# FlowEternal/multitask-hydranet

Hardware: AMD Instinct MI355X
Metric: images/sec (fwd+bwd) HydraNet @ default res, 1/2/4/8 MI355X; CPU-ref same run (higher is better)
Workload: dtype bf16; 1 GPU; full HydraNet (backbone + BiFPN + seg/det/lane heads + multitask loss), big cfg, fwd+loss+bwd; batch_per_gpu=16, global_batch=16, resolution=3x512x1024, parallelism=dp1, hipgraph=True

## Files before the change

include/hydranet_hip.h:

```cpp
#ifndef HYDRANET_HIP_H
#define HYDRANET_HIP_H

#ifdef __cplusplus
extern "C" {
#endif

typedef struct ihipStream_t* hipStream_t;


int hn_gconv_pack_diag(const float* w, void* wk, void* wd, int C, hipStream_t stream);
int hn_pack_weight(const float* w, void* wp, void* wt, int Cout, int Cin, int taps, hipStream_t stream);
int hn_pack_weight_ex(const float* w, void* wp, void* wt, int Cout, int Cin_total, int ci0, int Cin, int taps, int phase, const float* bias,
                      float* b_eff, hipStream_t stream);
int hn_phase_fold(const float* dw_eff, const float* dw1, const float* db_eff, float* dw, float* db, int K, int C0, int C1, hipStream_t stream);
int hn_pack_weights_batched(const long* jobs, int njobs, long total_blocks, const int* block_job, hipStream_t stream);
int hn_pack_small_batched(const long* jobs, const int* block_job, long total_blocks, hipStream_t stream);

int hn_conv_gemm_nt(const void* x0, const void* x1, int mode, int n_img, int H, int W, int C0, int C1, int ld0, int ld1, int up, long M,
                    const void* w, int Nout, int KP, int taps, const float* bias, int act, void* out, int out_f32, int ldc, long rpi,
                    long img_stride, float* psum, float* psq, hipStream_t stream);
int hn_nt_stat_rows(long M, int Nout);
int hn_nt_stat_tile(long M, int Nout);
int hn_direct_stat_rows(int n_img, int H, int W);
int hn_conv_gemm_nt_imgw(const void* x0, int ld0, long M, int C0, const void* w, long w_img_stride, long rows_per_image, int Nout, int KP,
                         const float* bias, int act, void* out, int ldc, const void* addend, int ld_add, hipStream_t stream);
int hn_scale_weight_gate(const void* wp, const float* gate, void* out, int N, int Cout, int C, int KP, hipStream_t stream);
int hn_conv_gemm_nt_lvl(const void* x0, int ld0, long M, int C0, const void* w, int Nout, int KP, const float* bias, int act, void* out,
                        int ldc, const float* coef, int nlev, const long* rows, hipStream_t stream);
int hn_conv_gemm_nt_lvlout(const void* x0, int ld0, long M, int C0, const void* w, int Nout, int KP, const float* bias, int act, float* out,
                           int ldc, long img_stride, int n_img, int nlev, const int* H, const int* W, int row_align, hipStream_t stream);

int hn_conv_gemm_nt_ex(const void* x0, const void* x1, int mode, int n_img, int H, int W, int C0, int C1, int ld0, int ld1, int up, long M,
                       const void* w, int Nout, int KP, int taps, const float* bias, int act, void* out, int out_f32, int ldc, long rpi,
                       long img_stride, float* psum, float* psq, const float* xscale, const float* xshift, const float* xgate, long xhw,
                       int xact, const void* addend, int ld_add, int add_mode, hipStream_t stream);
int hn_conv_gemm_nt_stat(const void* x0, const void* x1, int mode, int n_img, int H, int W, int C0, int C1, int ld0, int ld1, int up, long M,
                         const void* w, int Nout, int KP, int taps, const float* bias, int act, void* out, int out_f32, int ldc, long rpi,
                         long img_stride, float* psum, float* psq, const void* addend, int ld_add, int add_mode, int emode, const void* ez,
                         int ld_ez, const float* ecoef, hipStream_t stream);
int hn_conv_gemm_nt_stat3(const void* x0, int ld0, long M, int C0, const void* w, int Nout, int KP, void* out, int ldc, float* psum, float* psq,
                          const void* addend, int ld_add, const void* ez, int ld_ez, const void* ey, int ld_ey, const float* ecoef,
                          hipStream_t stream);
int hn_wgrad_plan(int mode, int n_img, int H, int W, long M, int Nout, int KP, int taps, int* splits, long* rows_per_split, long* ws_bytes);
int hn_conv_gemm_tn(const void* x0, const void* x1, int mode, int n_img, int H, int W, int C0, int C1, int ld0, int ld1, int up, long M,
                    const void* dz, int ldz, int Nout, int KP, int taps, float* workspace, float* dw, hipStream_t stream);


int hn_stem_fwd(const float* x, const float* w, void* z, void* patches, int N, int H, int W, hipStream_t stream);

int hn_gconv_pack(const float* w, void* wk, void* wd, int C, int flip, hipStream_t stream);
int hn_gconv_fwd(const void* in, int ldi, const void* wk, void* out, int ldo, int N, int Hi, int Wi, int C, int stride, hipStream_t stream);
int hn_gconv_dgrad_s2(const void* dz, int ldz, const void* wd, void* dx, int ldx, int N, int Hi, int Wi, int C, hipStream_t stream);
long hn_wgrad_chunks(long pixels, long items);
int hn_gconv_wgrad(const void* x, int ldx, const void* dz, int ldz, float* part, int N, int Hi, int Wi, int C, int stride,
                   hipStream_t stream);

int hn_dw_pack(const float* w, void* wk, void* wkf, int C, hipStream_t stream);
int hn_dwconv_fwd(const void* in, int ldi, const void* wk, void* out, int ldo, int N, int H, int W, int C, hipStream_t stream);
int hn_dwconv_fwd_levels(const void* in, int ldi, const void* wk, void* out, int ldo, int N, int C, int nlev, const int* H, const int* W,
                         int row_align, int accumulate, hipStream_t stream);
long hn_dwconv_wgrad_blocks(long strips, int C);
int hn_dwconv_wgrad(const void* x, int ldx, const void* dz, int ldz, float* part, int N, int H, int W, int C, hipStream_t stream);
int hn_dwconv_wgrad_levels(const void* x, int ldx, const void* dz, int ldz, float* part, int N, int C, int nlev, const int* H, const int* W,
                           int row_align, hipStream_t stream);
long hn_dwconv_bwd_blocks(long strips, int C);
long hn_dwconv_bwd_blocks_levels(int N, int C, int nlev, const int* H, const int* W);
int hn_dwconv_bwd_levels(const void* dz, int ldz, const void* x, int ldx, const void* wf, void* dx, int lddx, float* part, int N, int C,
                         int nlev, const int* H, const int* W, int row_align, int accumulate, hipStream_t stream);

int hn_maxpool_fwd(const void* in, int ldi, void* out, int ldo, int N, int H, int W, int C, int mode, hipStream_t stream);
int hn_maxpool_bwd(const void* in, int ldi, const void* dout, int ldd, void* dx, int ldx, const float* wscale, int N, int H, int W, int C,
                   int mode, hipStream_t stream);
int hn_maxpool_bwd2(const void* in, int ldi, const void* dout, int ldd, void* dx, int ldx, const float* wscale, void* arg_ws, int N, int H,
                    int W, int C, int mode, int accumulate, hipStream_t stream);

int hn_up2_fwd(const void* in, int ldi, void* out, int ldo, int N, int H, int W, int C, hipStream_t stream);
int hn_sum2x2(const void* g, int ldg, void* out, int ldo, const float* wscale, int N, int H, int W, int C, int accumulate, hipStream_t stream);

int hn_fuse_dweights(const float* pw, int blocks, const float* praw, int nw, float eps, float* dp, hipStream_t stream);
int hn_fuse_fwd(const void* const* in, const int* ld, const int* mode, const float* w, void* out, int ldo, int N, int H, int W, int C,
                hipStream_t stream);
int hn_fuse_fwd_raw(const void* const* in, const int* ld, const int* mode, const float* praw, int nw, float eps, float* wn, void* out, int ldo,
                    int N, int H, int W, int C, hipStream_t stream);
int hn_fuse_bwd_blocks(int N, int H, int W, int C);
int hn_fuse_bwd(const void* const* in, const int* ld, const int* mode, const float* w, const void* dout, int ldd, void* g, int ldg,
                void* const* din, const int* ldin, const int* acc, float* pw, int N, int H, int W, int C, hipStream_t stream);
int hn_fuse_bwd_arg(const void* const* in, const int* ld, const int* mode, const float* w, const void* dout, int ldd, void* g, int ldg,
                    void* const* din, const int* ldin, const int* acc, float* pw, void* const* arg_out, int N, int H, int W, int C,
                    hipStream_t stream);
int hn_maxpool_bwd_from_arg(const void* arg, const void* dout, int ldd, void* dx, int ldx, const float* wscale, int N, int H, int W, int C,
                            int mode, int accumulate, hipStream_t stream);

long hn_fold_ring_rows(int H, int W);
int hn_conv3x3_dgrad_fold(const void* dz, int ldz, int Cz, int n_img, int H, int W, const void* wt, int Nout, int KP, int phase_k, int clamp,
                          void* out, int ldo, const void* yprev, int ldy, void* ring, hipStream_t stream);
int hn_conv3x3_dgrad_fold_s2d(const void* dz, int ldz, int Cz, int n_img, int H, int W, const void* wt, int Nout, int KP, int phase_k, int clamp,
                              void* out, int ldo, void* out_s2d, int ld_s2d, const void* yprev, int ldy, void* ring, hipStream_t stream);
int hn_seg_fold(const void* dvp, int ldv, int c0, void* out, int ldo, const void* yprev, int ldy, int N, int H, int W, int C, int up,
                hipStream_t stream);

int hn_space_to_depth(const float* dy, void* out, int ldo, int N, int h, int w, int k, hipStream_t stream);

int hn_space_to_depth_blocks(int N, int h, int w, int k);
int hn_space_to_depth_bf16(const void* in, int ldi, void* out, int N, int h, int w, int k, float* psum, hipStream_t stream);

// ... 260 lines not shown
```

multitask_hydranet_amd/csrc/hn_gemm.hip:

```cpp
#include "hn_common.h"
#include <climits>

#ifdef HN_TUNING
#define HN_DBG(p) ((p).dbg)
#else
#define HN_DBG(p) 0
#endif

struct XSrc {
    const bf16* x0;
    const bf16* x1;
    int mode;
    int H, W;
    int Hi, Wi;
    int C0, C1;
    int ld0, ld1;
    int up;
    long M;
    int clamp;
    int diag;
};

__device__ __forceinline__ int border_idx(int v, int L, int clamp) {
    if (clamp == 2) return (v < 0 || v >= L) ? -1 : v;
// ... 610 lines not shown
    if (staged || want_stats) __syncthreads();
    if (want_stats && !e3 && tid < BC && c_blk + tid < p.Nout) {
        const float* red = reinterpret_cast<const float*>(smem + BP * BC * 2);
        float t1 = 0.f, t2 = 0.f;
#pragma unroll
        for (int k = 0; k < WGP; ++k) { t1 += red[(k * BC + tid) * 2]; t2 += red[(k * BC + tid) * 2 + 1]; }
        p.psum[(long)p_tile * p.Nout + c_blk + tid] = t1;
        if (p.psq) p.psq[(long)p_tile * p.Nout + c_blk + tid] = t2;
    }
    if (staged) {
        bf16* outp = reinterpret_cast<bf16*>(p.out);
        float e1[8], e2[8], emu[8], ers[8];
#pragma unroll
        for (int k = 0; k < 8; ++k) { e1[k] = 0.f; e2[k] = 0.f; emu[k] = 0.f; ers[k] = 0.f; }
        if (e3) {
            const int co = c_blk + (tid % NPC) * 8;
            if (co < p.Nout) {
#pragma unroll
                for (int k = 0; k < 8; ++k) { emu[k] = p.ecoef[2 * p.Nout + co + k]; ers[k] = p.ecoef[3 * p.Nout + co + k]; }
            }
        }
#pragma unroll
        for (int u = 0; u < NIT; ++u) {
            const int idx = tid + 256 * u;
            if (idx >= BP * NPC) break;
            const int row = idx / NPC, pc = idx % NPC;
            const long pix = p_blk + row;
            const int co = c_blk + pc * 8;
            if (pix < p.x.M && co < p.Nout) {
                bf16x8 v = *reinterpret_cast<const bf16x8*>(smem + row * (BC * 2) + (((pc ^ row) & (NPC - 1)) << 4));
                long orow = pix * p.ldc;
                if (p.rpi) {
                    const unsigned im = (unsigned)pix / (unsigned)p.rpi;
                    orow = (long)im * p.img_stride + (long)((unsigned)pix - im * (unsigned)p.rpi) * p.ldc;
                }
                if (p.addend && !p.add_pre) {
                    bool has = true;
                    bf16x8 a;
                    if (PRE) {
                        has = phas[u < PRE ? u : 0];
                        a = padd[u < PRE ? u : 0];
                    } else {
                        long arow = pix;
                        if (p.add_s2) {
                            const unsigned W = (unsigned)p.x.W, H = (unsigned)p.x.H;
                            const unsigned x = (unsigned)pix % W, t = (unsigned)pix / W;
                            const unsigned y = t % H, n = t / H;
                            has = !((x | y) & 1u);
                            arow = ((long)n * (H >> 1) + (y >> 1)) * (W >> 1) + (x >> 1);
                        }
                        a = has ? ld8(p.addend + arow * p.ld_add + co) : zero8();
                    }
                    if (has) {
#pragma unroll
                        for (int k = 0; k < 8; ++k) v[k] = f2bf(bf2f(v[k]) + bf2f(a[k]));
                    }
                }
                if (e3) {
                    const bf16x8 yv = PRE ? pey[u < PRE ? u : 0] : ld8(p.ey + pix * p.ld_ey + co);
                    const bf16x8 zv = PRE ? pzz[u < PRE ? u : 0] : ld8(p.ez + pix * p.ld_ez + co);
#pragma unroll
                    for (int k = 0; k < 8; ++k) {
                        const float g = bf2f(yv[k]) > 0.f ? bf2f(v[k]) : 0.f;
                        e1[k] += g;
                        e2[k] += g * (bf2f(zv[k]) - emu[k]) * ers[k];
                    }
                }
                *reinterpret_cast<bf16x8*>(outp + orow + co) = v;
            }
        }
        if (e3) {
            float* r3 = reinterpret_cast<float*>(smem + BP * BC * 2 + WGP * BC * 8);
            static_assert(BP * BC * 2 + WGP * BC * 8 + 256 * 16 * 4 <= R * KG * STAGE || BC < 64, "emode 3 scratch fits the operand ring");
#pragma unroll
            for (int k = 0; k < 8; ++k) { r3[tid * 16 + k] = e1[k]; r3[tid * 16 + 8 + k] = e2[k]; }
            __syncthreads();
            if (tid < BC && c_blk + tid < p.Nout) {
                const int pc = tid >> 3, k = tid & 7;
                float t1 = 0.f, t2 = 0.f;
                for (int j = 0; j < 256 / NPC; ++j) { t1 += r3[(j * NPC + pc) * 16 + k]; t2 += r3[(j * NPC + pc) * 16 + 8 + k]; }
                p.psum[(long)p_tile * p.Nout + c_blk + tid] = t1;
                p.psq[(long)p_tile * p.Nout + c_blk + tid] = t2;
            }
        }
    }
}

template <int BC, bool OUT_F32, bool PIPE, int XB = (PIPE ? 2 : 1)>
__global__ __launch_bounds__(512, 4) void conv3x3_direct_kernel(const GemmNT p) {
    constexpr int KC = PIPE ? 32 : 64;
    constexpr int NPP = KC / 8, PB = KC * 2;
    constexpr int XBUFS = XB, WBUFS = PIPE ? 4 : 2;
    constexpr int WCO = BC >= 64 ? 64 : BC;
    constexpr int WGC = BC / WCO, WGP = 8 / WGC, ROWS = 16 / WGP;
    constexpr int TC = WCO / 16, TP = ROWS;
    constexpr int PPIX = 18 * 18, XL = (PPIX * NPP + 511) / 512, WL = (BC * NPP + 511) / 512;
    constexpr bool PRE32 = PIPE && XB == 1;
    constexpr int XBYTES = PIPE ? XL * 512 * 16 : (PPIX * 128 + 1023) / 1024 * 1024, WBYTES = PRE32 ? BC * PB : (PIPE ? WL * 512 * 16 : BC * 128);
    extern __shared__ __attribute__((aligned(16))) char smem[];
    char* sXb = smem;
    char* sWb = smem + XBUFS * XBYTES;
    const int tid = threadIdx.x, lane = tid & 63, wave = __builtin_amdgcn_readfirstlane(tid >> 6);
    const int wc = wave / WGP, wp = wave % WGP;
    const XSrc& xs = p.x;
    const int ncy = (p.Nout + BC - 1) / BC;
    const int tx_n = (xs.W + 15) >> 4, ty_n = (xs.H + 15) >> 4;
    const int lid = xcd_remap(blockIdx.x, gridDim.x);
    unsigned long long* stampb = (HN_DBG(p) & 16) && (blockIdx.x & 63) == 0 && tid == 0
                                     ? reinterpret_cast<unsigned long long*>(p.dbg_buf) + (blockIdx.x >> 6) * 128 : nullptr;
    int stampi = 0;
    auto stamp = [&]() {
#ifdef HN_TUNING
        __builtin_amdgcn_sched_barrier(0);
        if (stampb && stampi < 128) stampb[stampi++] = __builtin_amdgcn_s_memtime();
        __builtin_amdgcn_sched_barrier(0);
#endif
    };
    stamp();
    const int npatch = gridDim.x / ncy;
    const int c_tile = p.tile_major ? lid / npatch : lid % ncy;
    int t = p.tile_major ? lid % npatch : lid / ncy;
    const int patch_id = t;
    const int tx = t % tx_n;
    t /= tx_n;
    const int ty = t % ty_n;
    const int n = t / ty_n;
    const int c_blk = c_tile * BC, oy0 = ty * 16, ox0 = tx * 16;
    const int org = xs.mode == 2 ? -1 : -2;
    const int Ctot = xs.C0 + xs.C1;
    const int NT = p.phase_mode ? 4 : 9;
    const int nchunk = xs.diag ? 1 : (p.KP + KC - 1) / KC, S = nchunk * NT;
    const int Ktot = 9 * p.KP;
    const int tile_phase = p.phase_mode == 1 ? c_blk / p.phase_span : 0;
    const int cpp = p.phase_mode == 2 ? p.phase_span / KC : 0;
    struct Cur { int chunk, ti, ph, cnt; };
    auto cur0 = [&]() { Cur c; c.chunk = 0; c.ti = 0; c.ph = tile_phase; c.cnt = 0; return c; };
    auto adv = [&](Cur& c) {
        if (++c.ti == NT) {
            c.ti = 0;
            ++c.chunk;
            if (p.phase_mode == 2 && ++c.cnt == cpp) { c.cnt = 0; ++c.ph; }
        }
    };
    auto tap_at = [&](const Cur& c) { return p.phase_mode ? ((c.ph >> 1) + (c.ti >> 1)) * 3 + (c.ph & 1) + (c.ti & 1) : c.ti; };
    const int xc0 = xs.diag ? c_blk : 0;
    float* sbias = reinterpret_cast<float*>(smem + XBUFS * XBYTES + ((!PIPE || PRE32) && p.wpre ? S : WBUFS) * WBYTES);
    if (tid < BC) sbias[tid] = (p.bias && c_blk + tid < p.Nout) ? p.bias[c_blk + tid] : 0.f;

    if (BC == 64 && !PIPE && xs.diag) {
#pragma unroll
        for (int i = 0; i < 2; ++i) {
            if (512 * i + 64 * wave < 9 * 64) {
                const int e = 512 * i + tid, tap = e >> 6, col = e & 63, co = c_blk + col;
                const bf16* src = co < p.Nout ? p.w + co * (9 * p.KP) + tap * 64 + (col >> 3) * 8 : g_zero_piece;
                glds16(src, smem + XBUFS * XBYTES + (512 * i + 64 * wave) * 16);
            }
        }
    }
    int* patch_src = reinterpret_cast<int*>(sbias + BC);
    if (tid < 36) {
        const bool isy = tid < 18;
        const int k = isy ? tid : tid - 18, L = isy ? xs.Hi : xs.Wi;
        int g = (isy ? oy0 : ox0) + org + k;
        if (xs.mode == 2) g = border_idx(g, L, xs.clamp);
        else g = (g >= 0 && g < L) ? g : -1;
        patch_src[tid] = g;
// ... 2147 lines not shown
    const XSrc& x = p.x;
    const long npatch = (long)cdiv(x.W, 16) * cdiv(x.H, 16) * n_img;
    if (x.clamp == 1 && !x.diag && !out_f32 && p.d2s == 64 && p.phase_mode == 1 && p.phase_span == 64 && p.taps == 9 && p.KP == 64 && x.C0 == 64 &&
        x.C1 == 0 && p.Nout == 256 && !p.psum && !p.addend && (p.act == HN_ACT_ELU || p.act == HN_ACT_NONE) && (x.ld0 & 7) == 0 &&
        (p.ldc & 7) == 0 && p.ldc >= 64 && aligned16(p.out) && g_hn_knob[11] != 3 && npatch >= 1024) {
        SegPhase q;
        q.x = x.x0; q.ldx = x.ld0; q.N = n_img; q.H = x.H; q.W = x.W; q.w = p.w; q.bias = p.bias; q.out = (bf16*)p.out; q.ldc = p.ldc;
        q.act = p.act; q.npatch = (int)npatch;
        q.ppw = cdiv(npatch, 64);
        const int grid = 4 * cdiv(npatch, q.ppw);
        const size_t lds = 2 * (size_t)((18 * 18 * 8 + 63) / 64) * 1024 + 256 * 128;
        static std::atomic<unsigned long long> optin_sp{0};
        if (!lds_optin(optin_sp, {(const void*)seg_phase64_conv_kernel})) return HN_ERR_LAUNCH;
        hipLaunchKernelGGL(seg_phase64_conv_kernel, dim3(grid), dim3(512), lds, st, q);
        HN_LAUNCH_CHECK();
    }
    if (x.clamp == 1 && !x.diag && out_f32 && p.d2s && p.taps == 9 && p.KP == 64 && x.C0 == 64 && x.C1 == 0 && p.Nout == 4 * p.d2s &&
        p.Nout <= 32 && !p.psum && !p.addend && p.phase_mode == 0 && p.act == HN_ACT_NONE && (x.ld0 & 7) == 0 && ((32 * p.d2s) & 3) == 0 &&
        ((2 * x.W * p.d2s) & 3) == 0 && aligned16(p.out) && g_hn_knob[11] != 3 && npatch >= 1024) {
        SegOut q;
        q.x = x.x0; q.ldx = x.ld0; q.N = n_img; q.H = x.H; q.W = x.W; q.w = p.w; q.Nout = p.Nout; q.k = p.d2s; q.bias = p.bias;
        q.out = p.amax ? nullptr : (float*)p.out; q.amax = p.amax; q.npatch = (int)npatch;
        q.ppw = cdiv(npatch, 256);
        const int grid = cdiv(npatch, q.ppw);
        const size_t lds = 2 * (size_t)((18 * 18 * 8 + 63) / 64) * 1024 + (size_t)32 * 32 * p.d2s * 4;
        static std::atomic<unsigned long long> optin_so{0};
        if (!lds_optin(optin_so, {(const void*)seg_out_conv_kernel<true>, (const void*)seg_out_conv_kernel<false>})) return HN_ERR_LAUNCH;
        if (p.amax) hipLaunchKernelGGL(seg_out_conv_kernel<true>, dim3(grid), dim3(512), lds, st, q);
        else hipLaunchKernelGGL(seg_out_conv_kernel<false>, dim3(grid), dim3(512), lds, st, q);
        HN_LAUNCH_CHECK();
    }
    HN_CHECK_ARG(x.Wi < 8192 && x.Hi < 32768);
    int bc = x.diag ? 64 : (p.Nout <= 16 ? 16 : (p.Nout <= 32 ? 32 : (p.Nout <= 64 ? 64 : 128)));
    if (p.phase_mode == 1 && p.phase_span < bc) bc = 64;
    const bool staged_ok = (p.ldc & 7) == 0 && (p.Nout & 7) == 0 && aligned16(p.out) && (!p.d2s || ((p.d2s & 7) == 0 && p.Nout % bc == 0));
    if (bc >= 64 && !out_f32 && !staged_ok) {
        if (x.diag) return HN_ERR_UNSUPPORTED;
        bc = 32;
    }
    dim3 grid((unsigned)(cdiv(p.Nout, bc) * cdiv(x.W, 16) * cdiv(x.H, 16) * n_img));
    const int nsteps = p.phase_mode ? 4 : 9;
    p.wpre = (!x.diag && p.KP <= 64 && (size_t)nsteps * bc * 128 <= 32768 && g_hn_knob[11] != 2) ? 1 : 0;
    const bool narrow = bc == 64 && !out_f32 && !x.diag && !p.wpre && p.KP <= 32 && nsteps == 9 && g_hn_knob[18] == 0;
    if (narrow) p.wpre = 1;
#ifdef HN_TUNING
    const bool pipe = narrow || (g_direct_pipe && bc >= 64 && !out_f32 && !x.diag && !p.wpre && p.KP > 64);
#else
    const bool pipe = narrow;
#endif
    const size_t lds = narrow ? (size_t)(((18 * 18 * 4 + 511) / 512) * 512 * 16) + 9 * (size_t)(64 * 64)
                     : pipe ? (size_t)2 * (((18 * 18 * 4 + 511) / 512) * 512 * 16) + 4 * (size_t)(512 * 16)
                            : (size_t)((18 * 18 * 128 + 1023) / 1024 * 1024) + (p.wpre ? nsteps : 2) * (size_t)bc * 128;
    const size_t lds_bias = (size_t)bc * 4 + 36 * 4;
    static std::atomic<unsigned long long> optin{0};
    if (!lds_optin(optin, {(const void*)conv3x3_direct_kernel<16, true, false>, (const void*)conv3x3_direct_kernel<16, false, false>,
                           (const void*)conv3x3_direct_kernel<32, true, false>, (const void*)conv3x3_direct_kernel<32, false, false>,
                           (const void*)conv3x3_direct_kernel<64, true, false>, (const void*)conv3x3_direct_kernel<64, false, false>,
                           (const void*)conv3x3_direct_kernel<128, true, false>, (const void*)conv3x3_direct_kernel<128, false, false>}))
        return HN_ERR_LAUNCH;
    if (narrow) {
        hipLaunchKernelGGL((conv3x3_direct_kernel<64, false, true, 1>), grid, dim3(512), lds + lds_bias, st, p);
        HN_LAUNCH_CHECK();
    }
#ifdef HN_TUNING
    static std::atomic<unsigned long long> optin_pipe{0};
    if (pipe) {
        if (!lds_optin(optin_pipe, {(const void*)conv3x3_direct_kernel<64, false, true>, (const void*)conv3x3_direct_kernel<128, false, true>}))
            return HN_ERR_LAUNCH;
        if (bc == 64) hipLaunchKernelGGL((conv3x3_direct_kernel<64, false, true>), grid, dim3(512), lds + lds_bias, st, p);
        else hipLaunchKernelGGL((conv3x3_direct_kernel<128, false, true>), grid, dim3(512), lds + lds_bias, st, p);
        HN_LAUNCH_CHECK();
    }
#endif
#define DIRECT_CASE(BC_) \
    if (bc == BC_) { \
        if (out_f32) hipLaunchKernelGGL((conv3x3_direct_kernel<BC_, true, false>), grid, dim3(512), lds + lds_bias, st, p); \
        else hipLaunchKernelGGL((conv3x3_direct_kernel<BC_, false, false>), grid, dim3(512), lds + lds_bias, st, p); \
    }
    DIRECT_CASE(16) DIRECT_CASE(32) DIRECT_CASE(64) DIRECT_CASE(128)
#undef DIRECT_CASE
    HN_LAUNCH_CHECK();
}

static int run_gemm_nt(GemmNT& p, int n_img, bool out_f32, hipStream_t st) {
    const XSrc& x = p.x;
    const int Nout = p.Nout, KP = p.KP, taps = p.taps;
    const long M = x.M;
    HN_CHECK_ARG(x.x0 && p.w && p.out && M > 0 && Nout > 0 && KP > 0 && (KP & 31) == 0 && taps >= 1 && taps <= 9);
    HN_CHECK_ARG(!p.xscale || (p.xshift && x.mode <= 1 && !out_f32 && x.C1 == 0 && (!p.xgate || p.xhw > 0)));
    HN_CHECK_ARG(p.phase_mode == 0 || ((x.mode == 3 || x.clamp == 1) && p.phase_span >= 64 && p.phase_span % 64 == 0 && !p.psum && !p.rpi));
    HN_CHECK_ARG(!p.addend || p.add_pre || (!out_f32 && (Nout & 7) == 0 && (p.ldc & 7) == 0 && (p.ld_add & 7) == 0 && p.rpi == 0 && x.mode <= 1 &&
                                            aligned16(p.out) && aligned16(p.addend)));
    HN_CHECK_ARG(!p.addend || !p.add_pre || ((x.mode <= 1 || p.phase_mode == 1) && p.rpi == 0 && (p.ld_add & 3) == 0));
    HN_CHECK_ARG((x.C0 & 7) == 0 && (x.C1 & 7) == 0 && (x.ld0 & 7) == 0 && (x.C1 == 0 || (x.x1 && (x.ld1 & 7) == 0)));
    HN_CHECK_ARG(x.mode >= 0 && x.mode <= 3 && (!x.clamp || (x.up == 0 && x.C1 == 0)));
    HN_CHECK_ARG(x.diag ? (KP == 64 && Nout == x.C0 && !p.rpi) : x.C0 + x.C1 <= KP);
    HN_CHECK_ARG(x.mode == 0 || (long)n_img * x.H * x.W == M);
    HN_CHECK_ARG(x.mode < 2 ? taps == 1 : taps == 9);
    HN_CHECK_ARG(x.mode != 2 || x.clamp || (x.H >= 2 && x.W >= 2));
    HN_CHECK_ARG(p.add_s2 == 0 || (p.add_s2 == 1 && p.addend && !p.add_pre && p.ld_add > 0 && x.mode == 0 && !(x.H & 1) && !(x.W & 1) &&
                                   (long)n_img * x.H * x.W == M && M < (1L << 32)));
    HN_CHECK_ARG(!p.lcoef || (x.mode == 0 && taps == 1 && !p.psum && !p.xscale));
    HN_CHECK_ARG(!p.lo_n || (x.mode == 0 && taps == 1 && out_f32 && !p.psum && !p.xscale && p.rpi == 0 && !p.addend && M < (1L << 32)));
    HN_CHECK_ARG(p.w_rpi == 0 || (x.mode == 0 && taps == 1 && !p.xscale && p.w_rpi % 128 == 0 && M < (1L << 32)));
    HN_CHECK_ARG(p.emode != 3 || (x.mode == 0 && taps == 1 && p.psum && p.psq && !out_f32 && p.addend && !p.add_pre && p.ld_add > 0 && !p.add_s2 &&
                                   (Nout & 7) == 0 && (p.ldc & 7) == 0 && p.rpi == 0 && aligned16(p.out) && small_tile(M, Nout)));
    HN_CHECK_ARG(!p.d2s || (x.clamp == 1 && (out_f32 || p.phase_mode == 1) && p.rpi == 0 && !p.psum && Nout == 4 * p.d2s));
    p.tile_major = g_hn_knob[11] == 1 ? 1 : 0;
    p.dbg = (int)g_hn_knob[14];
    p.dbg_buf = reinterpret_cast<unsigned long long*>(g_hn_knob[15]);
    if (x.mode >= 2 && (!p.psum || x.diag) && !p.rpi) return launch_direct(p, n_img, out_f32, st);
    if (p.xscale) {
#ifdef HN_TUNING
        if (small_tile(M, Nout)) return launch_nt_xf<64, 64, 2, 2>(p, st);
        switch (pick_bc(Nout)) {
            case 16: return launch_nt_xf<16, 128, 1, 4>(p, st);
            case 32: return launch_nt_xf<32, 128, 1, 4>(p, st);
            case 64: return launch_nt_xf<64, 128, 2, 2>(p, st);
            default: return launch_nt_xf<128, 128, 2, 2>(p, st);
        }
#else
        return HN_ERR_UNSUPPORTED;
#endif
    }
    if (small_tile(M, Nout)) {
        if (x.mode <= 1 && taps == 1 && KP >= (g_hn_knob[6] > 1 ? g_hn_knob[6] : 512) && g_hn_knob[6] != 1 && !g_nt_force_r)
            return launch_nt_r<64, 64, 2, 2, 2, 2>(p, out_f32, st);
        return launch_nt<64, 64, 2, 2>(p, out_f32, st);
    }
    switch (pick_bc(Nout)) {
        case 16: return launch_nt<16, 128, 1, 4>(p, out_f32, st);
        case 32: return launch_nt<32, 128, 1, 4>(p, out_f32, st);
        case 64: return launch_nt<64, 128, 2, 2>(p, out_f32, st);
        default: return launch_nt<128, 128, 2, 2>(p, out_f32, st);
    }
}

extern "C" int hn_conv_gemm_nt(const void* x0, const void* x1, int mode, int n_img, int H, int W, int C0, int C1, int ld0, int ld1,
                               int up, long M, const void* w, int Nout, int KP, int taps, const float* bias, int act, void* out,
                               int out_f32, int ldc, long rpi, long img_stride, float* psum, float* psq, hipStream_t st) {
    GemmNT p = nt_conv(x0, x1, mode, H, W, C0, C1, ld0, ld1, up, M, w, Nout, KP, taps, bias, act, out, ldc, rpi, img_stride, psum, psq);
    return run_gemm_nt(p, n_img, out_f32, st);
}

extern "C" int hn_conv_gemm_nt_imgw(const void* x0, int ld0, long M, int C0, const void* w, long w_img_stride, long rows_per_image, int Nout,
                                    int KP, const float* bias, int act, void* out, int ldc, const void* addend, int ld_add, hipStream_t st) {
    HN_CHECK_ARG(rows_per_image > 0 && rows_per_image % 128 == 0 && M % rows_per_image == 0 && w_img_stride >= (long)Nout * KP);
    HN_CHECK_ARG(!addend || ld_add > 0);
    GemmNT p = nt_rows(x0, ld0, M, C0, w, Nout, KP, bias, act, out, ldc);
    p.w_img_stride = w_img_stride; p.w_rpi = (unsigned)rows_per_image;
    if (addend) { p.addend = (const bf16*)addend; p.ld_add = ld_add; p.add_pre = 1; }
    return run_gemm_nt(p, 0, false, st);
}

extern "C" int hn_conv_gemm_nt_lvl(const void* x0, int ld0, long M, int C0, const void* w, int Nout, int KP, const float* bias, int act,
                                   void* out, int ldc, const float* coef, int nlev, const long* rows, hipStream_t st) {
    HN_CHECK_ARG(coef && rows && nlev >= 1 && nlev <= HN_MAX_LEVELS);
    GemmNT p = nt_rows(x0, ld0, M, C0, w, Nout, KP, bias, act, out, ldc);
    p.lcoef = coef; p.ln = nlev;
    for (int l = 0; l < nlev; ++l) {
        HN_CHECK_ARG(rows[l] > 0 && rows[l] % 128 == 0);
        p.lrow[l + 1] = p.lrow[l] + rows[l];
    }
    HN_CHECK_ARG(p.lrow[nlev] == M);
    return run_gemm_nt(p, 0, false, st);
}

extern "C" int hn_conv_gemm_nt_lvlout(const void* x0, int ld0, long M, int C0, const void* w, int Nout, int KP, const float* bias, int act,
                                      float* out, int ldc, long img_stride, int n_img, int nlev, const int* H, const int* W, int row_align,
                                      hipStream_t st) {
    HN_CHECK_ARG(out && H && W && n_img > 0 && nlev >= 1 && nlev <= HN_MAX_LEVELS && row_align > 0 && row_align % 128 == 0 && img_stride >= 0);
    GemmNT p = nt_rows(x0, ld0, M, C0, w, Nout, KP, bias, act, out, ldc);
    p.img_stride = img_stride;
    p.ln = nlev; p.lo_n = n_img;
    unsigned pix = 0;
    for (int l = 0; l < nlev; ++l) {
        HN_CHECK_ARG(H[l] > 0 && W[l] > 0);
        const long real = (long)n_img * H[l] * W[l];
        p.lrow[l + 1] = p.lrow[l] + (real + row_align - 1) / row_align * row_align;
        p.lo_hw[l] = (unsigned)(H[l] * W[l]);
        p.lo_pix[l] = pix;
        pix += p.lo_hw[l];
    }
    HN_CHECK_ARG(p.lrow[nlev] == M);
    return run_gemm_nt(p, 0, true, st);
}

__global__ __launch_bounds__(256) void scale_weight_gate_kernel(const bf16* wp, const float* gate, bf16* out, int N, int Cout, int C, int KP) {
    const unsigned k8n = (unsigned)KP >> 3;
    const unsigned total = (unsigned)N * (unsigned)Cout * k8n;
    for (unsigned idx = blockIdx.x * 256u + threadIdx.x; idx < total; idx += gridDim.x * 256u) {
        const unsigned t = idx / k8n, k8 = idx - t * k8n;
        const unsigned n = t / (unsigned)Cout, co = t - n * (unsigned)Cout;
        const bf16x8 v = ld8(wp + (long)co * KP + k8 * 8);
        bf16x8 o;
#pragma unroll
        for (int j = 0; j < 8; ++j) {
            const int k = (int)k8 * 8 + j;
            o[j] = f2bf(k < C ? bf2f(v[j]) * gate[(long)n * C + k] : 0.f);
        }
        st8(out + ((long)n * Cout + co) * KP + k8 * 8, o);
    }
}
extern "C" int hn_scale_weight_gate(const void* wp, const float* gate, void* out, int N, int Cout, int C, int KP, hipStream_t st) {
    HN_CHECK_ARG(wp && gate && out && N > 0 && Cout > 0 && C > 0 && C <= KP && (KP & 31) == 0 && (long)N * Cout * (KP >> 3) < (1L << 31));
    long b = ((long)N * Cout * (KP >> 3) + 255) / 256;
    if (b > 4096) b = 4096;
// ... 620 lines not shown
```

Before: 984.4 images/sec.

## Add streaming register-resident GEMM kernel for tall skinny 1x1 convolutions

Adds a specialized kernel for 1x1 convolutions with small K (up to 128) and Nout up to 128 on large row counts. The whole weight tile stays in LDS, activations are streamed through registers with a 4-deep buffer-load prefetch, and bias, activation, optional addend and per-tile BN statistics are fused in. run_gemm_nt routes eligible shapes with at least 65536 rows here instead of the generic tiled NT path. The aim is to make these memory-bound layers approach streaming bandwidth. The stats reduction layout differs from the generic path and must still match the expected per-tile partial sums.

Result: no change. 984.2 images/sec (-0.0%).

```diff
diff --git a/include/hydranet_hip.h b/include/hydranet_hip.h
--- a/include/hydranet_hip.h
+++ b/include/hydranet_hip.h
@@ -21,6 +21,10 @@
                     long img_stride, float* psum, float* psq, hipStream_t stream);
 int hn_nt_stat_rows(long M, int Nout);
 int hn_nt_stat_tile(long M, int Nout);
+int hn_conv_gemm_nt_stream(const void* x0, int ld0, long M, int C0, const void* w, int Nout, int KP, const float* bias, int act, void* out,
+                           int ldc, const void* addend, int ld_add, float* psum, float* psq, hipStream_t stream);
+int hn_nt_stream_plan(long M, int C0, int Nout, int KP, int flags);
+int hn_nt_stream_span(long M, int Nout, int KP, int flags);
 int hn_direct_stat_rows(int n_img, int H, int W);
 int hn_conv_gemm_nt_imgw(const void* x0, int ld0, long M, int C0, const void* w, long w_img_stride, long rows_per_image, int Nout, int KP,
                          const float* bias, int act, void* out, int ldc, const void* addend, int ld_add, hipStream_t stream);
diff --git a/multitask_hydranet_amd/csrc/hn_gemm.hip b/multitask_hydranet_amd/csrc/hn_gemm.hip
--- a/multitask_hydranet_amd/csrc/hn_gemm.hip
+++ b/multitask_hydranet_amd/csrc/hn_gemm.hip
@@ -716,6 +716,154 @@
                 p.psum[(long)p_tile * p.Nout + c_blk + tid] = t1;
                 p.psq[(long)p_tile * p.Nout + c_blk + tid] = t2;
             }
+        }
+    }
+}
+
+template <typename SRD>
+__device__ __forceinline__ bf16x8 bld8(const SRD srd, unsigned off) {
+    return __builtin_bit_cast(bf16x8, __builtin_amdgcn_raw_buffer_load_b128(srd, (int)off, 0, 0));
+}
+
+struct GemmNTStream {
+    const bf16* x; int ld0, C0; long M;
+    const bf16* w; int Nout, KP;
+    const float* bias; int act;
+    bf16* out; int ldc;
+    const bf16* addend; int ld_add;
+    float* psum; float* psq;
+    int sh;
+    int groups;
+};
+
+template <int KC, int NT, bool STATS>
+__global__ __launch_bounds__(256, 2) void gemm_nt_stream_kernel(const GemmNTStream p) {
+    static_assert(NT % 2 == 0 && KC >= 1 && KC <= 4, "cout tiles come in pairs (one 16-byte piece per lane), K <= 128");
+    constexpr int NJ = NT / 2, NP = NT * 16, DEPTH = 4, GP = (STATS && NT == 8) ? 1 : 2;
+    extern __shared__ __attribute__((aligned(16))) char smem[];
+    bf16x8* sw = reinterpret_cast<bf16x8*>(smem);
+    float* sbias = reinterpret_cast<float*>(smem + NT * KC * 1024);
+    float* red = sbias + NP;
+    const int tid = threadIdx.x, lane = tid & 63, wave = __builtin_amdgcn_readfirstlane(tid >> 6);
+    const int px = lane & 15, g = lane >> 4;
+    const int lid = xcd_remap(blockIdx.x, gridDim.x);
+    const long row0 = (long)lid * p.groups * 64;
+
+    const auto xsrd = __builtin_amdgcn_make_buffer_rsrc(const_cast<bf16*>(p.x), 0, (int)(unsigned)(((p.M - 1) * p.ld0 + p.C0) * 2), 0x00020000);
+    const auto wsrd = __builtin_amdgcn_make_buffer_rsrc(const_cast<bf16*>(p.w), 0, p.Nout * p.KP * 2, 0x00020000);
+    constexpr int SLOTS = NT * KC * 64, WPT = (SLOTS + 255) / 256;
+    bf16x8 wreg[WPT];
+#pragma unroll
+    for (int u = 0; u < WPT; ++u) {
+        const int idx = tid + 256 * u, frag = idx >> 6, l = idx & 63, i = frag / KC, kc = frag - i * KC, a = l & 15;
+        const int co = (((i >> 1) * 4 + (a >> 2)) << 3) + (i & 1) * 4 + (a & 3);
+        wreg[u] = bld8(wsrd, (idx < SLOTS && co < p.Nout) ? (unsigned)(co * p.KP + kc * 32 + 8 * (l >> 4)) * 2u : 0xffffffffu);
+    }
+    const auto bsrd = __builtin_amdgcn_make_buffer_rsrc(const_cast<float*>(p.bias), 0, p.bias ? p.Nout * 4 : 0, 0x00020000);
+    const float breg = __builtin_bit_cast(float, __builtin_amdgcn_raw_buffer_load_b32(bsrd, tid < p.Nout ? tid * 4 : -1, 0, 0));
+
+    bf16x8 xb[DEPTH][KC];
+    auto issue = [&](const int s, const int b) {
+        const long row = row0 + (long)b * 64 + s * 16 + px;
+        const bool rv = row < p.M && b < p.groups;
+        const unsigned off = ((unsigned)row * (unsigned)p.ld0 + 8u * g) * 2u;
+#pragma unroll
+        for (int kc = 0; kc < KC; ++kc) xb[s][kc] = bld8(xsrd, (rv && kc * 32 + 8 * g < p.C0) ? off + kc * 64u : 0xffffffffu);
+    };
+#pragma unroll
+    for (int s = 0; s < DEPTH; ++s) issue(s, wave);
+    __builtin_amdgcn_sched_barrier(0);
+#pragma unroll
+    for (int u = 0; u < WPT; ++u)
+        if (tid + 256 * u < SLOTS) sw[tid + 256 * u] = wreg[u];
+    if (tid < NP) sbias[tid] = breg;
+    __syncthreads();
+
+    float s1[STATS ? NJ : 1][8], s2[STATS ? NJ : 1][8];
+#pragma unroll
+    for (int j = 0; j < (STATS ? NJ : 1); ++j)
+#pragma unroll
+        for (int k = 0; k < 8; ++k) { s1[j][k] = 0.f; s2[j][k] = 0.f; }
+
+    for (int b = wave; b < p.groups; b += 4) {
+#pragma unroll
+        for (int h = 0; h < DEPTH; h += GP) {
+            f32x4 acc[GP][NT];
+#pragma unroll
+            for (int e = 0; e < GP; ++e)
+#pragma unroll
+                for (int i = 0; i < NT; ++i) acc[e][i] = (f32x4){0.f, 0.f, 0.f, 0.f};
+#pragma unroll
+            for (int kc = 0; kc < KC; ++kc) {
+#pragma unroll
+                for (int i = 0; i < NT; ++i) {
+                    const bf16x8 af = sw[(i * KC + kc) * 64 + lane];
+#pragma unroll
+                    for (int e = 0; e < GP; ++e) acc[e][i] = __builtin_amdgcn_mfma_f32_16x16x32_bf16(af, xb[h + e][kc], acc[e][i], 0, 0, 0);
+                }
+            }
+#pragma unroll
+            for (int e = 0; e < GP; ++e) issue(h + e, b + 4);
+            __builtin_amdgcn_sched_barrier(0);
+#pragma unroll
+            for (int e = 0; e < GP; ++e) {
+                const long row = row0 + (long)b * 64 + (h + e) * 16 + px;
+                const bool rv = row < p.M;
+#pragma unroll
+                for (int j = 0; j < NJ; ++j) {
+                    const int co = (j * 4 + g) * 8;
+                    const f32x4 bl = *reinterpret_cast<const f32x4*>(sbias + co), bh = *reinterpret_cast<const f32x4*>(sbias + co + 4);
+                    float v[8];
+#pragma unroll
+                    for (int r = 0; r < 4; ++r) { v[r] = acc[e][2 * j][r] + bl[r]; v[4 + r] = acc[e][2 * j + 1][r] + bh[r]; }
+                    if constexpr (STATS) {
+#pragma unroll
+                        for (int k = 0; k < 8; ++k) {
+                            const float q = rv ? bfround(v[k]) : 0.f;
+                            s1[j][k] += q;
+                            s2[j][k] += q * q;
+                        }
+                    }
+                    act_fwd_n(v, p.act);
+                    bf16x8 t;
+#pragma unroll
+                    for (int k = 0; k < 8; ++k) t[k] = f2bf(v[k]);
+                    if (rv && co < p.Nout) {
+                        if (p.addend) {
+                            const bf16x8 a = ld8(p.addend + row * p.ld_add + co);
+#pragma unroll
+                            for (int k = 0; k < 8; ++k) t[k] = f2bf(bf2f(t[k]) + bf2f(a[k]));
+                        }
+                        st8(p.out + row * p.ldc + co, t);
+                    }
+                }
+            }
+        }
+        if constexpr (STATS) {
+#pragma unroll
+            for (int j = 0; j < NJ; ++j) {
+                const int co = (j * 4 + g) * 8;
+#pragma unroll
+                for (int k = 0; k < 8; ++k) {
+                    const float t1 = row16_sum(s1[j][k]), t2 = row16_sum(s2[j][k]);
+                    if (px == 0) *reinterpret_cast<float2*>(red + ((long)b * NP + co + k) * 2) = make_float2(t1, t2);
+                    s1[j][k] = 0.f;
+                    s2[j][k] = 0.f;
+                }
+            }
+        }
+    }
+    if constexpr (STATS) {
+        __syncthreads();
+        const int bpt = p.sh >> 6, nt = p.groups / bpt;
+        const long tile0 = row0 / p.sh;
+        for (int idx = tid; idx < nt * NP; idx += 256) {
+            const int tl = idx / NP, c = idx - tl * NP;
+            if (c >= p.Nout || (tile0 + tl) * p.sh >= p.M) continue;
+            float t1 = 0.f, t2 = 0.f;
+            for (int k = 0; k < bpt; ++k) { t1 += red[((tl * bpt + k) * NP + c) * 2]; t2 += red[((tl * bpt + k) * NP + c) * 2 + 1]; }
+            p.psum[(tile0 + tl) * p.Nout + c] = t1;
+            if (p.psq) p.psq[(tile0 + tl) * p.Nout + c] = t2;
         }
     }
 }
@@ -3029,6 +3177,104 @@
     HN_LAUNCH_CHECK();
 }
 
+#define HN_STREAM_MIN_ROWS 65536
+#define HN_STREAM_STATS 1
+#define HN_STREAM_ADDEND 2
+#define HN_STREAM_F32 4
+#define HN_STREAM_OTHER 8
+
+static int stream_nt_of(int kc, int Nout) {
+    if (Nout <= 0 || Nout > 128 || kc < 1 || kc > 4) return 0;
+    const int nt = Nout <= 32 ? 2 : (Nout <= 64 ? 4 : 8);
+    switch (kc * 16 + nt) {
+        case 1 * 16 + 2: case 1 * 16 + 4:
+        case 2 * 16 + 2: case 2 * 16 + 4: case 2 * 16 + 8:
+        case 3 * 16 + 8:
+        case 4 * 16 + 4: case 4 * 16 + 8: return nt;
+        default: return 0;
+    }
+}
+
+static bool stream_shape_ok(long M, int C0, int Nout, int KP) {
+    return M > 0 && KP > 0 && KP <= 128 && (KP & 31) == 0 && C0 > 0 && C0 <= KP && (C0 & 7) == 0 && Nout > 0 && Nout <= 128 && (Nout & 7) == 0 &&
+           stream_nt_of(KP >> 5, Nout) != 0;
+}
+
+static bool stream_eligible(const GemmNT& p, bool out_f32) {
+    const XSrc& x = p.x;
+    return x.mode == 0 && p.taps == 1 && x.C1 == 0 && !x.diag && !x.clamp && x.x0 && p.w && p.out && stream_shape_ok(x.M, x.C0, p.Nout, p.KP) &&
+           (x.ld0 & 7) == 0 && x.ld0 >= x.C0 && x.M * x.ld0 < (1L << 30) && aligned16(x.x0) && aligned16(p.w) && !out_f32 && (p.ldc & 7) == 0 && p.ldc >= p.Nout && aligned16(p.out) &&
+           !p.xscale && !p.rpi && !p.w_rpi && !p.lcoef && !p.lo_n && !p.d2s && !p.fold && !p.phase_mode && !p.add_s2 && !p.amax && p.emode == 0 &&
+           (!p.addend || (!p.add_pre && (p.ld_add & 7) == 0 && p.ld_add >= p.Nout && aligned16(p.addend))) && (!p.psq || p.psum);
+}
+
+static size_t stream_lds(int kc, int nt, int groups, bool stats) {
+    return (size_t)nt * kc * 1024 + (size_t)nt * 16 * 4 + (stats ? (size_t)groups * nt * 16 * 8 : 0);
+}
+static int stream_groups(long M, int kc, int nt, bool stats) {
+    int g = 4;
+#ifdef HN_TUNING
+    if (g_hn_knob[19] >= 4) return (int)(g_hn_knob[19] & ~3L);
+#endif
+    while (g < 16 && cdiv(M, (long)g * 64) > 1024 && stream_lds(kc, nt, 2 * g, stats) <= 64 * 1024) g *= 2;
+    return g;
+}
+
+extern "C" int hn_nt_stream_span(long M, int Nout, int KP, int flags) {
+    const int kc = KP >> 5, nt = stream_nt_of(kc, Nout);
+    if (M <= 0 || !nt) return 0;
+    return 64 * stream_groups(M, kc, nt, (flags & HN_STREAM_STATS) != 0);
+}
+
+extern "C" int hn_nt_stream_plan(long M, int C0, int Nout, int KP, int flags) {
+    if (flags & (HN_STREAM_F32 | HN_STREAM_OTHER)) return 0;
+#ifdef HN_TUNING
+    if (g_hn_knob[19] == 1) return 0;
+#endif
+    return stream_shape_ok(M, C0, Nout, KP) && M >= HN_STREAM_MIN_ROWS ? 1 : 0;
+}
+
+template <int KC, int NT>
+static int launch_stream(const GemmNTStream& q, size_t lds, hipStream_t st) {
+    const dim3 grid(cdiv(q.M, (long)q.groups * 64));
+    if (q.psum) hipLaunchKernelGGL((gemm_nt_stream_kernel<KC, NT, true>), grid, dim3(256), lds, st, q);
+    else hipLaunchKernelGGL((gemm_nt_stream_kernel<KC, NT, false>), grid, dim3(256), lds, st, q);
+    HN_LAUNCH_CHECK();
+}
+
+static int run_gemm_nt_stream(const GemmNT& p, hipStream_t st) {
+    GemmNTStream q;
+    q.x = p.x.x0; q.ld0 = p.x.ld0; q.C0 = p.x.C0; q.M = p.x.M;
+    q.w = p.w; q.Nout = p.Nout; q.KP = p.KP; q.bias = p.bias; q.act = p.act;
+    q.out = (bf16*)p.out; q.ldc = p.ldc; q.addend = p.addend; q.ld_add = p.ld_add; q.psum = p.psum; q.psq = p.psq;
+    const int kc = p.KP >> 5, nt = stream_nt_of(kc, p.Nout);
+    q.sh = hn_nt_stat_tile(q.M, q.Nout);
+    q.groups = stream_groups(q.M, kc, nt, q.psum != nullptr);
+    const size_t lds = stream_lds(kc, nt, q.groups, q.psum != nullptr);
+    if (lds > 64 * 1024 || cdiv(q.M, (long)q.groups * 64) <= 0) return HN_ERR_UNSUPPORTED;
+    switch (kc * 16 + nt) {
+        case 1 * 16 + 2: return launch_stream<1, 2>(q, lds, st);
+        case 1 * 16 + 4: return launch_stream<1, 4>(q, lds, st);
+        case 2 * 16 + 2: return launch_stream<2, 2>(q, lds, st);
+        case 2 * 16 + 4: return launch_stream<2, 4>(q, lds, st);
+        case 2 * 16 + 8: return launch_stream<2, 8>(q, lds, st);
+        case 3 * 16 + 8: return launch_stream<3, 8>(q, lds, st);
+        case 4 * 16 + 4: return launch_stream<4, 4>(q, lds, st);
+        case 4 * 16 + 8: return launch_stream<4, 8>(q, lds, st);
+        default: return HN_ERR_UNSUPPORTED;
+    }
+}
+
+extern "C" int hn_conv_gemm_nt_stream(const void* x0, int ld0, long M, int C0, const void* w, int Nout, int KP, const float* bias, int act,
+                                      void* out, int ldc, const void* addend, int ld_add, float* psum, float* psq, hipStream_t st) {
+    HN_CHECK_ARG(x0 && w && out && M > 0 && act >= HN_ACT_NONE && act <= HN_ACT_SIGMOID && (!addend || ld_add > 0));
+    GemmNT p = nt_rows(x0, ld0, M, C0, w, Nout, KP, bias, act, out, ldc);
+    p.psum = psum; p.psq = psq;
+    if (addend) { p.addend = (const bf16*)addend; p.ld_add = ld_add; }
+    HN_CHECK_ARG(stream_eligible(p, false));
+    return run_gemm_nt_stream(p, st);
+}
+
 static int run_gemm_nt(GemmNT& p, int n_img, bool out_f32, hipStream_t st) {
     const XSrc& x = p.x;
     const int Nout = p.Nout, KP = p.KP, taps = p.taps;
@@ -3070,6 +3316,8 @@
         return HN_ERR_UNSUPPORTED;
 #endif
     }
+    if (stream_eligible(p, out_f32) && hn_nt_stream_plan(M, x.C0, Nout, KP, (p.psum ? HN_STREAM_STATS : 0) | (p.addend ? HN_STREAM_ADDEND : 0)))
+        return run_gemm_nt_stream(p, st);
     if (small_tile(M, Nout)) {
         if (x.mode <= 1 && taps == 1 && KP >= (g_hn_knob[6] > 1 ? g_hn_knob[6] : 512) && g_hn_knob[6] != 1 && !g_nt_force_r)
             return launch_nt_r<64, 64, 2, 2, 2, 2>(p, out_f32, st);
```
